# VISION-SJTU/USOT

Hardware: AMD Instinct MI355X
Metric: tracker FPS (255x255 search, ResNet-50) (higher is better)
Workload: dtype f32; 1 GPU; configs[1]: batch=1 ResNet-50(layer3)+neck, fused depthwise xcorr, cls/reg/memory heads (N_q=7), decode + PrRoIPool, fp32, 1 stream per GPU; search=255, template=127, streams=1, streams_per_gpu=1, weights=synthetic seed 0 (calibrated BN), no broadcast 0 B, hipgraph=True, devices_visible=1, sessions=1, hip_streams=1

## Files before the change

### usot_amd/csrc/smallm_f32.hip

```cpp
#include <hip/hip_runtime.h>
#include <stdint.h>
#include "usot_hip.h"
#include "common.h"

#ifndef USOT_RING
#define USOT_RING 8
#endif

namespace {

typedef float f32x4 __attribute__((ext_vector_type(4)));
typedef double f64x4 __attribute__((ext_vector_type(4)));
typedef unsigned int u32x4_t __attribute__((ext_vector_type(4)));
typedef unsigned int u32x2_t __attribute__((ext_vector_type(2)));
typedef _Float16 f16x8_t __attribute__((ext_vector_type(8)));

struct PwF {
    const float *t2, *w3p, *b3, *res, *w1p, *b1;
    float *y, *t, *ws;
    int M, act2;
    int parts = 0;
    const float *tbias = nullptr;
    int rparts = 0;
    const float *rbias = nullptr;
    int *ovf = nullptr;
};

template <int CBW, int RS, int RT, int PF, int BLO = 0>
struct GemmRing {
    static constexpr int N = CBW * RS;
    static_assert(BLO == 0 || (RS % 4 == 0 && PF % 2 == 0), "split-fp16: whole 64-k blocks, fragments in pairs");
    static_assert(PF <= N, "ring deeper than the work");
    f32x4 ring[PF];
    __device__ __forceinline__ f32x4 frag(const f32x4 *__restrict__ wf, int cb0, int r0, int n) const
    {
        return wf[((cb0 + n / RS) * RT + r0 + n % RS) * 64];
    }
    __device__ __forceinline__ void prefetch(const f32x4 *__restrict__ wf, int cb0, int r0)
    {
#pragma unroll
        for (int n = 0; n < PF; ++n) ring[n] = frag(wf, cb0, r0, n);
    }
    __device__ __forceinline__ void run(const f32x4 *__restrict__ wf, const float *bs, int cb0, int r0, f32x4 (&acc)[CBW])
    {
        constexpr int G = 4;
        const f32x4 zero = {0.f, 0.f, 0.f, 0.f};
        f32x4 part[CBW][2];
        BlockTotal tot[CBW];
#pragma unroll
        for (int u = 0; u < CBW; ++u) { part[u][0] = part[u][1] = zero; tot[u].clear(); }
        if constexpr (BLO > 0) {
            auto h = [](const f32x4 &v) { return __builtin_bit_cast(f16x8_t, v); };
#pragma unroll
            for (int n = 0; n < N; n += 2) {
                const int step = (r0 + n % RS) >> 1;
                const f32x4 bh = *(const f32x4 *)(bs + step * 16), bl = *(const f32x4 *)(bs + BLO + step * 16);
                const f32x4 ah = ring[n % PF], al = ring[(n + 1) % PF];
                if (n + PF < N) ring[n % PF] = frag(wf, cb0, r0, n + PF);
                if (n + 1 + PF < N) ring[(n + 1) % PF] = frag(wf, cb0, r0, n + 1 + PF);
                const int u = n / RS, rr = n % RS, g = rr / G, s = g & 1;
                const bool first = rr % G == 0;
                if (first && g >= 2) tot[u].add(part[u][s]);
                part[u][s] = __builtin_amdgcn_mfma_f32_16x16x32_f16(h(al), h(bh), first ? zero : part[u][s], 0, 0, 0);
                part[u][s] = __builtin_amdgcn_mfma_f32_16x16x32_f16(h(ah), h(bl), part[u][s], 0, 0, 0);
                part[u][s] = __builtin_amdgcn_mfma_f32_16x16x32_f16(h(ah), h(bh), part[u][s], 0, 0, 0);
            }
        } else {
#pragma unroll
        for (int n = 0; n < N; ++n) {
            const f32x4 b = *(const f32x4 *)(bs + (r0 + n % RS) * 16);
            const f32x4 a = ring[n % PF];
            if (n + PF < N) ring[n % PF] = frag(wf, cb0, r0, n + PF);
            const int u = n / RS, rr = n % RS, g = rr / G, s = g & 1;
            const bool first = rr % G == 0;
            if (first && g >= 2) tot[u].add(part[u][s]);
#pragma unroll
            for (int c = 0; c < 4; ++c)
                part[u][s] = __builtin_amdgcn_mfma_f32_16x16x4f32(a[c], b[c], (first && c == 0) ? zero : part[u][s], 0, 0, 0);
        }
        }
#pragma unroll
        for (int u = 0; u < CBW; ++u) {
            constexpr int GL = (RS - 1) / G;
            if (GL >= 1) tot[u].add(part[u][(GL & 1) ^ 1]);
            tot[u].add(part[u][GL & 1]);
            acc[u] = tot[u].get();
        }
    }
};

template <int CBW, int RS, int RT, int BLO = 0>
__device__ __forceinline__ void gemm_blocks(const f32x4 *__restrict__ wf, const float *bs, int cb0, int r0, f32x4 (&acc)[CBW])
{
    GemmRing<CBW, RS, RT, (CBW * RS < USOT_RING ? CBW * RS : USOT_RING), BLO> g;
    g.prefetch(wf, cb0, r0);
    g.run(wf, bs, cb0, r0, acc);
}

__device__ __forceinline__ void store_split4(char *row, int k, int plane, f32x4 v)
{
    v *= 8.0f;
    const uint32_t hi0 = usot_pack2_lp<true>(v[0], v[1]), hi1 = usot_pack2_lp<true>(v[2], v[3]);
    const usot_f16x2 h0 = __builtin_bit_cast(usot_f16x2, hi0), h1 = __builtin_bit_cast(usot_f16x2, hi1);
    const uint32_t lo0 = usot_pack2_lp<true>(v[0] - (float)h0[0], v[1] - (float)h0[1]);
    const uint32_t lo1 = usot_pack2_lp<true>(v[2] - (float)h1[0], v[3] - (float)h1[1]);
    *(u32x2_t *)(row + k * 2) = u32x2_t{hi0, hi1};
    *(u32x2_t *)(row + plane + k * 2) = u32x2_t{lo0, lo1};
}

__device__ __forceinline__ void note_not_finite(int *ovf, const f32x4 &a)
{
    if (!ovf) return;
    bool bad = false;
#pragma unroll
    for (int e = 0; e < 4; ++e) bad |= !(__builtin_fabsf(a[e]) <= 3.4028234664e38f);
    if (bad) __hip_atomic_store(ovf, 1, __ATOMIC_RELAXED, __HIP_MEMORY_SCOPE_AGENT);
}

template <int CM, int COT, int CN, int S, bool H16 = false>
__device__ __forceinline__ void pair_tail(const PwF &p, const float *Xs, float *Ys, float *Ps, int pt, int sl)
{
    constexpr int NW = 8, BM = 16;
    constexpr int CO = COT / S;
    constexpr int R1 = CM / 16, NB1 = CO / 16;
    constexpr int R2 = CO / 16, NB2 = CN / 16, R2T = COT / 16;
    constexpr int CBW1 = NB1 / NW;
    constexpr int KS = NB2 >= NW ? 1 : NW / NB2;
    constexpr int CBW2 = NB2 >= NW ? NB2 / NW : 1;
    constexpr int RS2 = R2 / KS;
    static_assert(NB1 % NW == 0 && (NB2 % NW == 0 || NW % NB2 == 0) && R2 % KS == 0, "shape");
    static_assert(S == 1 || KS == 1, "the sliced form keeps GEMM2's k range of a workgroup in one piece");
    constexpr int XP = CM + 4, YP = CO + 4, PP = CN + 4;
    const int tid = threadIdx.x, lane = tid & 63, wave = tid >> 6;
    const int l15 = lane & 15, quad = lane >> 4;
    const int m = pt * BM + l15;
    const bool mok = m < p.M;

    {
        f32x4 rr[CBW1], bb[CBW1], sc[H16 ? CBW1 : 1];
#pragma unroll
        for (int u = 0; u < CBW1; ++u) {
            const int cog = sl * CO + (wave * CBW1 + u) * 16 + quad * 4;
            if constexpr (H16) sc[u] = *(const f32x4 *)(p.w3p + (long)COT * CM + cog);
            rr[u] = mok ? *(const f32x4 *)(p.res + (long)m * COT + cog) : f32x4{0.f, 0.f, 0.f, 0.f};
            if (p.rparts > 1 && mok) {
                for (int q = 1; q < p.rparts; ++q) rr[u] += *(const f32x4 *)(p.res + ((long)q * p.M + m) * COT + cog);
                rr[u] += *(const f32x4 *)(p.rbias + cog);
            }
            bb[u] = *(const f32x4 *)(p.b3 + cog);
        }
        f32x4 acc[CBW1];
        gemm_blocks<CBW1, R1, R1, H16 ? CM / 2 : 0>((const f32x4 *)p.w3p + lane + (long)sl * NB1 * R1 * 64, Xs + l15 * XP + quad * 4, wave * CBW1, 0, acc);
#pragma unroll
        for (int u = 0; u < CBW1; ++u) {
            const int co = (wave * CBW1 + u) * 16 + quad * 4;
            if constexpr (H16) {
                acc[u] *= sc[u];
                note_not_finite(p.ovf, acc[u]);
            }
            f32x4 v = acc[u] + bb[u] + rr[u];
#pragma unroll
            for (int e = 0; e < 4; ++e) v[e] = fmaxf(v[e], 0.f);
            if (mok) *(f32x4 *)(p.y + (long)m * COT + sl * CO + co) = v;
            if constexpr (H16) store_split4((char *)(Ys + l15 * YP), co, CO * 2, v);
            else *(f32x4 *)(Ys + l15 * YP + co) = v;
        }
    }
    __syncthreads();

    const int ksl = KS > 1 ? wave / NB2 : 0;
    const int cb0 = KS > 1 ? wave % NB2 : wave * CBW2;
    f32x4 acc[CBW2];
    gemm_blocks<CBW2, RS2, R2T, H16 ? CO / 2 : 0>((const f32x4 *)p.w1p + lane + (long)sl * R2 * 64, Ys + l15 * YP + quad * 4, cb0, ksl * RS2, acc);
    if constexpr (H16) {
#pragma unroll
        for (int u = 0; u < CBW2; ++u) {
            acc[u] *= *(const f32x4 *)(p.w1p + (long)CN * COT + (cb0 + u) * 16 + quad * 4);
            note_not_finite(p.ovf, acc[u]);
        }
    }
    if constexpr (KS > 1) {
        const int cn = cb0 * 16 + quad * 4;
        if (ksl > 0) *(f32x4 *)(Ps + ((ksl - 1) * BM + l15) * PP + cn) = acc[0];
        __syncthreads();
        if (ksl > 0) return;
#pragma unroll
        for (int s = 1; s < KS; ++s) acc[0] += *(const f32x4 *)(Ps + ((s - 1) * BM + l15) * PP + cn);
    }
    if constexpr (S > 1) {
        const long bytes = (long)S * p.M * CN * 4;
        const __amdgpu_buffer_rsrc_t rs = __builtin_amdgcn_make_buffer_rsrc((void *)p.ws, 0, (int)(bytes > 0x7fffffffL ? 0x7fffffffL : bytes), 0x00020000);
#pragma unroll
        for (int u = 0; u < CBW2; ++u)
            if (mok) __builtin_amdgcn_raw_buffer_store_b128(__builtin_bit_cast(u32x4_t, acc[u]), rs,
                                                            (int)((((long)sl * p.M + m) * CN + (cb0 + u) * 16 + quad * 4) * 4), 0, 16);
        asm volatile("s_waitcnt vmcnt(0)" ::: "memory");
        __syncthreads();
        int *flag = (int *)Ps;
        if (tid == 0) {
            int *cnt = (int *)(p.ws + (long)S * p.M * CN) + pt;
            const int ticket = __hip_atomic_fetch_add(cnt, 1, __ATOMIC_RELAXED, __HIP_MEMORY_SCOPE_AGENT);
            const int last = ticket == S - 1;
            if (last) __hip_atomic_store(cnt, 0, __ATOMIC_RELAXED, __HIP_MEMORY_SCOPE_AGENT);
            *flag = last;
        }
        __syncthreads();
        if (!*flag || !mok) return;
#pragma unroll
        for (int u = 0; u < CBW2; ++u) {
            f32x4 sum = {0.f, 0.f, 0.f, 0.f};
#pragma unroll
            for (int q = 0; q < S; ++q)
                sum += __builtin_bit_cast(f32x4, __builtin_amdgcn_raw_buffer_load_b128(rs, (int)((((long)q * p.M + m) * CN + (cb0 + u) * 16 + quad * 4) * 4), 0, 16));
            acc[u] = sum;
        }
    }
#pragma unroll
    for (int u = 0; u < CBW2; ++u) {
        const int cn = (cb0 + u) * 16 + quad * 4;
        f32x4 v = acc[u] + *(const f32x4 *)(p.b1 + cn);
        if (p.act2 == USOT_ACT_RELU) {
#pragma unroll
            for (int e = 0; e < 4; ++e) v[e] = fmaxf(v[e], 0.f);
        }
        if (mok) *(f32x4 *)(p.t + (long)m * CN + cn) = v;
    }
}

template <int CN, int KSG> constexpr int ps_floats() { return KSG > 1 ? (KSG - 1) * 16 * (CN + 4) : 16; }

template <int CM, int COT, int CN, int S = 1, bool H16 = false>
__global__ __launch_bounds__(512) void pw_pair_f32_kernel(const PwF p)
{
    constexpr int NW = 8, BM = 16, XP = CM + 4, NB2 = CN / 16, KS = NB2 >= NW ? 1 : NW / NB2;
    __shared__ __attribute__((aligned(16))) float Xs[BM * XP];
    __shared__ __attribute__((aligned(16))) float Ys[BM * (COT / S + 4)];
    __shared__ __attribute__((aligned(16))) float Ps[ps_floats<CN, KS>()];
    const int tid = threadIdx.x;
    const int pt = S > 1 ? (int)blockIdx.x / S : (int)blockIdx.x, sl = S > 1 ? (int)blockIdx.x % S : 0;
    const int bm0 = pt * BM;
    if (p.parts > 1) {
        const long slab = (long)p.M * CM;
        for (int i = tid; i < BM * (CM / 4); i += NW * 64) {
            const int row = i / (CM / 4), c4 = i - row * (CM / 4);
            f32x4 v = {0.f, 0.f, 0.f, 0.f};
            if (bm0 + row < p.M) {
                const float *src = p.t2 + (long)(bm0 + row) * CM + c4 * 4;
                v = *(const f32x4 *)src;
                for (int q = 1; q < p.parts; ++q) v += *(const f32x4 *)(src + q * slab);
                v += *(const f32x4 *)(p.tbias + c4 * 4);
#pragma unroll
                for (int e = 0; e < 4; ++e) v[e] = fmaxf(v[e], 0.f);
            }
            if constexpr (H16) store_split4((char *)(Xs + row * XP), c4 * 4, CM * 2, v);
            else *(f32x4 *)(Xs + row * XP + c4 * 4) = v;
        }
    } else {
        for (int i = tid; i < BM * (CM / 4); i += NW * 64) {
            const int row = i / (CM / 4), c4 = i - row * (CM / 4);
            f32x4 v = {0.f, 0.f, 0.f, 0.f};
            if (bm0 + row < p.M) v = *(const f32x4 *)(p.t2 + (long)(bm0 + row) * CM + c4 * 4);
            if constexpr (H16) store_split4((char *)(Xs + row * XP), c4 * 4, CM * 2, v);
            else *(f32x4 *)(Xs + row * XP + c4 * 4) = v;
        }
    }
    __syncthreads();
    pair_tail<CM, COT, CN, S, H16>(p, Xs, Ys, Ps, pt, sl);
}

struct PwT {
    PwF pair;
    const float *x, *w2p, *b2;
    int H, W, OH, OW, pad_h, pad_w, dil_h, dil_w;
};

template <int CIN, int CM, int COT, int CN>
__global__ __launch_bounds__(512) void pw_triple_f32_kernel(const PwT q)
{
    constexpr int NW = 8, BM = 16, TAPS = 9, K0 = TAPS * CIN, RT0 = K0 / 16, NB0 = CM / 16;
    constexpr int KS0 = NW / NB0, RS0 = RT0 / KS0;
    static_assert(NB0 <= NW && NW % NB0 == 0 && RT0 % KS0 == 0, "conv2: one column block per wave group");
    constexpr int XP0 = K0 + 4, XP = CM + 4, NB2 = CN / 16, KS2 = NB2 >= NW ? 1 : NW / NB2;
    constexpr int PSF = ps_floats<CM, KS0>() > ps_floats<CN, KS2>() ? ps_floats<CM, KS0>() : ps_floats<CN, KS2>();
    extern __shared__ __attribute__((aligned(16))) float ldst[];
    float *X0 = ldst;
    float *Xs = X0 + BM * XP0;
    float *Ys = Xs + BM * XP;
    float *Ps = Ys + BM * (COT + 4);
    __shared__ int pix[BM][3];
    const PwF &p = q.pair;
    const int tid = threadIdx.x, lane = tid & 63, wave = tid >> 6;
    const int l15 = lane & 15, quad = lane >> 4;
    const int pt = blockIdx.x, bm0 = pt * BM;
    const int cb = wave % NB0, ksl = wave / NB0;
    const f32x4 *wf = (const f32x4 *)q.w2p + lane;
    GemmRing<1, RS0, RT0, (RS0 < USOT_RING ? RS0 : USOT_RING)> g;
    g.prefetch(wf, cb, ksl * RS0);
    if (tid < BM) {
        const int mm = bm0 + tid;
        if (mm < p.M) {
            const int P = q.OH * q.OW, n = mm / P, r = mm - n * P, oh = r / q.OW;
            pix[tid][0] = n * q.H;
            pix[tid][1] = oh - q.pad_h;
            pix[tid][2] = (r - oh * q.OW) - q.pad_w;
        } else {
            pix[tid][0] = -1;
        }
    }
    __syncthreads();
    for (int i = tid; i < BM * TAPS * (CIN / 4); i += NW * 64) {
        const int c4 = i % (CIN / 4), t = (i / (CIN / 4)) % TAPS, row = i / (TAPS * (CIN / 4));
        f32x4 v = {0.f, 0.f, 0.f, 0.f};
        if (pix[row][0] >= 0) {
            const int ih = pix[row][1] + (t / 3) * q.dil_h, iw = pix[row][2] + (t % 3) * q.dil_w;
            if ((unsigned)ih < (unsigned)q.H && (unsigned)iw < (unsigned)q.W)
                v = *(const f32x4 *)(q.x + ((long)(pix[row][0] + ih) * q.W + iw) * CIN + c4 * 4);
        }
        *(f32x4 *)(X0 + row * XP0 + t * CIN + c4 * 4) = v;
    }
    const f32x4 b2 = *(const f32x4 *)(q.b2 + cb * 16 + quad * 4);
    __syncthreads();
    f32x4 acc[1];
    g.run(wf, X0 + l15 * XP0 + quad * 4, cb, ksl * RS0, acc);
    if constexpr (KS0 > 1) {
        if (ksl > 0) *(f32x4 *)(Ps + ((ksl - 1) * BM + l15) * (CM + 4) + cb * 16 + quad * 4) = acc[0];
        __syncthreads();
        if (ksl == 0) {
#pragma unroll
            for (int s2 = 1; s2 < KS0; ++s2) acc[0] += *(const f32x4 *)(Ps + ((s2 - 1) * BM + l15) * (CM + 4) + cb * 16 + quad * 4);
        }
    }
    if (ksl == 0) {
        f32x4 v = acc[0] + b2;
#pragma unroll
        for (int e = 0; e < 4; ++e) v[e] = fmaxf(v[e], 0.f);
        *(f32x4 *)(Xs + l15 * XP + cb * 16 + quad * 4) = v;
    }
    __syncthreads();
    pair_tail<CM, COT, CN, 1>(p, Xs, Ys, Ps, pt, 0);
}

template <int CM, int CO, int CN, int S = 1, bool H16 = false> int launch(hipStream_t s, const PwF &p)
{
    hipLaunchKernelGGL((pw_pair_f32_kernel<CM, CO, CN, S, H16>), dim3(((p.M + 15) / 16) * S), dim3(512), 0, s, p);
    return hipGetLastError() == hipSuccess ? USOT_OK : USOT_ELAUNCH;
}

template <int CIN, int CM, int CO, int CN> int launch_triple(hipStream_t s, const PwT &q)
{
    const int usot_dv = usot_device_slot();
    if (usot_dv < 0) return USOT_ESTATE;
    constexpr int NB2 = CN / 16, KS2 = NB2 >= 8 ? 1 : 8 / NB2, KS0 = 8 / (CM / 16);
    constexpr int PSF = ps_floats<CM, KS0>() > ps_floats<CN, KS2>() ? ps_floats<CM, KS0>() : ps_floats<CN, KS2>();
    const size_t lds = (size_t)(16 * (9 * CIN + 4) + 16 * (CM + 4) + 16 * (CO + 4) + PSF) * sizeof(float);
    static bool raised_d[USOT_MAX_DEV] = {};
    bool &raised = raised_d[usot_dv];
    if (lds > 64 * 1024 && !raised) {
        if (hipFuncSetAttribute((const void *)pw_triple_f32_kernel<CIN, CM, CO, CN>, hipFuncAttributeMaxDynamicSharedMemorySize, (int)lds) != hipSuccess)
            return USOT_ELAUNCH;
        raised = true;
    }
    hipLaunchKernelGGL((pw_triple_f32_kernel<CIN, CM, CO, CN>), dim3((q.pair.M + 15) / 16), dim3(512), lds, s, q);
    return hipGetLastError() == hipSuccess ? USOT_OK : USOT_ELAUNCH;
}

int slices(int M, int CM, int CN)
{
    if (CM == 128 && CN == 128 && M <= 2 * 961) return 4;
    if (CM == 256 && CN == 256 && M <= 1200) return 4;
    return 1;
}

struct Pw1 {
    const float *x, *wp, *b, *res;
    float *y;
    int M, act;
};

template <int K, int N, int S, int PFD = USOT_RING>
__global__ __launch_bounds__(512) void pw_single_f32_kernel(const Pw1 p)
{
    constexpr int NW = 8, BM = 16;
    constexpr int RT = K / 16, NB = N / 16 / S;
    constexpr int KS = NB >= NW ? 1 : NW / NB, CBW = NB >= NW ? NB / NW : 1, RS = RT / KS;
    static_assert((NB % NW == 0 || NW % NB == 0) && RT % KS == 0, "shape");
    constexpr int XP = K + 4, PP = NB * 16 + 4;
    extern __shared__ __attribute__((aligned(16))) float lds1[];
    float *Xs = lds1;
    float *Ps = lds1 + BM * XP;

    const int tid = threadIdx.x, lane = tid & 63, wave = tid >> 6;
    const int l15 = lane & 15, quad = lane >> 4;
    const int pt = (int)blockIdx.x / S, sl = (int)blockIdx.x % S;
    const int bm0 = pt * BM, m = bm0 + l15;
    const bool mok = m < p.M;
    const int ksl = KS > 1 ? wave / NB : 0;
    const int cb0 = KS > 1 ? wave % NB : wave * CBW;
    const f32x4 *wf = (const f32x4 *)p.wp + lane + (long)sl * NB * RT * 64;
    GemmRing<CBW, RS, RT, (CBW * RS < PFD ? CBW * RS : PFD)> g;
    g.prefetch(wf, cb0, ksl * RS);
    for (int i = tid; i < BM * (K / 4); i += NW * 64) {
        const int row = i / (K / 4), c4 = i - row * (K / 4);
        f32x4 v = {0.f, 0.f, 0.f, 0.f};
        if (bm0 + row < p.M) v = *(const f32x4 *)(p.x + (long)(bm0 + row) * K + c4 * 4);
        *(f32x4 *)(Xs + row * XP + c4 * 4) = v;
    }
    f32x4 rr[CBW], bb[CBW];
#pragma unroll
    for (int u = 0; u < CBW; ++u) {
        const int n = (sl * NB + cb0 + u) * 16 + quad * 4;
        rr[u] = (mok && p.res && ksl == 0) ? *(const f32x4 *)(p.res + (long)m * N + n) : f32x4{0.f, 0.f, 0.f, 0.f};
        bb[u] = *(const f32x4 *)(p.b + n);
    }
    __syncthreads();
    f32x4 acc[CBW];
    g.run(wf, Xs + l15 * XP + quad * 4, cb0, ksl * RS, acc);
    if constexpr (KS > 1) {
        if (ksl > 0) *(f32x4 *)(Ps + ((ksl - 1) * BM + l15) * PP + cb0 * 16 + quad * 4) = acc[0];
        __syncthreads();
        if (ksl > 0) return;
#pragma unroll
        for (int s2 = 1; s2 < KS; ++s2) acc[0] += *(const f32x4 *)(Ps + ((s2 - 1) * BM + l15) * PP + cb0 * 16 + quad * 4);
    }
#pragma unroll
    for (int u = 0; u < CBW; ++u) {
        f32x4 v = acc[u] + bb[u] + rr[u];
        if (p.act == USOT_ACT_RELU) {
#pragma unroll
            for (int e = 0; e < 4; ++e) v[e] = fmaxf(v[e], 0.f);
        }
        if (mok) *(f32x4 *)(p.y + (long)m * N + (sl * NB + cb0 + u) * 16 + quad * 4) = v;
    }
}

template <int K, int N, int S> int launch1(hipStream_t s, const Pw1 &p)
{
    const int usot_dv = usot_device_slot();
    if (usot_dv < 0) return USOT_ESTATE;
    constexpr int NB = N / 16 / S, KS = NB >= 8 ? 1 : 8 / NB;
    const size_t lds = (size_t)(16 * (K + 4) + (KS > 1 ? (KS - 1) * 16 * (NB * 16 + 4) : 0)) * sizeof(float);
    if (lds > 64 * 1024) {
        static bool raised_d[USOT_MAX_DEV] = {};
    bool &raised = raised_d[usot_dv];
        if (!raised) {
            if (hipFuncSetAttribute((const void *)pw_single_f32_kernel<K, N, S>, hipFuncAttributeMaxDynamicSharedMemorySize, (int)lds) != hipSuccess)
                return USOT_ELAUNCH;
            raised = true;
        }
    }
    hipLaunchKernelGGL((pw_single_f32_kernel<K, N, S>), dim3(((p.M + 15) / 16) * S), dim3(512), lds, s, p);
    return hipGetLastError() == hipSuccess ? USOT_OK : USOT_ELAUNCH;
}

struct PwC {
    const float *x, *wp, *b, *res;
    float *y;
    int M, H, W, OH, OW, pad_h, pad_w, dil_h, dil_w, act;
};

template <int CIN, int N, int S>
__global__ __launch_bounds__(512) void stream_conv3x3_f32_kernel(const PwC p)
{
    constexpr int NW = 8, BM = 16, TAPS = 9, K = TAPS * CIN;
    constexpr int RT = K / 16, NB = N / 16 / S;
    constexpr int KS = NB >= NW ? 1 : NW / NB, CBW = NB >= NW ? NB / NW : 1, RS = RT / KS;
    static_assert((NB % NW == 0 || NW % NB == 0) && RT % KS == 0, "shape");
    constexpr int XP = K + 4, PP = NB * 16 + 4;
    extern __shared__ __attribute__((aligned(16))) float ldsc[];
    float *Xs = ldsc;
    float *Ps = ldsc + BM * XP;
    __shared__ int pix[BM][3];

    const int tid = threadIdx.x, lane = tid & 63, wave = tid >> 6;
    const int l15 = lane & 15, quad = lane >> 4;
    const int pt = (int)blockIdx.x / S, sl = (int)blockIdx.x % S;
    const int bm0 = pt * BM, m = bm0 + l15;
    const bool mok = m < p.M;
    const int ksl = KS > 1 ? wave / NB : 0;
    const int cb0 = KS > 1 ? wave % NB : wave * CBW;
    const f32x4 *wf = (const f32x4 *)p.wp + lane + (long)sl * NB * RT * 64;
    GemmRing<CBW, RS, RT, (CBW * RS < USOT_RING ? CBW * RS : USOT_RING)> g;
    g.prefetch(wf, cb0, ksl * RS);
    if (tid < BM) {
        const int mm = bm0 + tid;
        if (mm < p.M) {
            const int P = p.OH * p.OW, n = mm / P, r = mm - n * P, oh = r / p.OW;
            pix[tid][0] = n * p.H;
            pix[tid][1] = oh - p.pad_h;
            pix[tid][2] = (r - oh * p.OW) - p.pad_w;
        } else {
            pix[tid][0] = -1;
        }
    }
    __syncthreads();
    for (int i = tid; i < BM * TAPS * (CIN / 4); i += NW * 64) {
        const int c4 = i % (CIN / 4), t = (i / (CIN / 4)) % TAPS, row = i / (TAPS * (CIN / 4));
        f32x4 v = {0.f, 0.f, 0.f, 0.f};
        if (pix[row][0] >= 0) {
            const int ih = pix[row][1] + (t / 3) * p.dil_h, iw = pix[row][2] + (t % 3) * p.dil_w;
            if ((unsigned)ih < (unsigned)p.H && (unsigned)iw < (unsigned)p.W)
                v = *(const f32x4 *)(p.x + ((long)(pix[row][0] + ih) * p.W + iw) * CIN + c4 * 4);
        }
        *(f32x4 *)(Xs + row * XP + t * CIN + c4 * 4) = v;
    }
    f32x4 rr[CBW], bb[CBW];
#pragma unroll
    for (int u = 0; u < CBW; ++u) {
        const int n = (sl * NB + cb0 + u) * 16 + quad * 4;
        rr[u] = (mok && p.res && ksl == 0) ? *(const f32x4 *)(p.res + (long)m * N + n) : f32x4{0.f, 0.f, 0.f, 0.f};
        bb[u] = *(const f32x4 *)(p.b + n);
    }
    __syncthreads();
    f32x4 acc[CBW];
    g.run(wf, Xs + l15 * XP + quad * 4, cb0, ksl * RS, acc);
    if constexpr (KS > 1) {
        if (ksl > 0) *(f32x4 *)(Ps + ((ksl - 1) * BM + l15) * PP + cb0 * 16 + quad * 4) = acc[0];
        __syncthreads();
        if (ksl > 0) return;
#pragma unroll
        for (int s2 = 1; s2 < KS; ++s2) acc[0] += *(const f32x4 *)(Ps + ((s2 - 1) * BM + l15) * PP + cb0 * 16 + quad * 4);
    }
#pragma unroll
    for (int u = 0; u < CBW; ++u) {
        f32x4 v = acc[u] + bb[u] + rr[u];
        if (p.act == USOT_ACT_RELU) {
#pragma unroll
            for (int e = 0; e < 4; ++e) v[e] = fmaxf(v[e], 0.f);
        }
        if (mok) *(f32x4 *)(p.y + (long)m * N + (sl * NB + cb0 + u) * 16 + quad * 4) = v;
    }
}

template <int CIN, int N, int S> int launch3(hipStream_t s, const PwC &p)
{
    const int usot_dv = usot_device_slot();
    if (usot_dv < 0) return USOT_ESTATE;
    constexpr int K = 9 * CIN, NB = N / 16 / S, KS = NB >= 8 ? 1 : 8 / NB;
    const size_t lds = (size_t)(16 * (K + 4) + (KS > 1 ? (KS - 1) * 16 * (NB * 16 + 4) : 0)) * sizeof(float);
    static bool raised_d[USOT_MAX_DEV] = {};
    bool &raised = raised_d[usot_dv];
    if (lds > 64 * 1024 && !raised) {
        if (hipFuncSetAttribute((const void *)stream_conv3x3_f32_kernel<CIN, N, S>, hipFuncAttributeMaxDynamicSharedMemorySize, (int)lds) != hipSuccess)
            return USOT_ELAUNCH;
        raised = true;
    }
    hipLaunchKernelGGL((stream_conv3x3_f32_kernel<CIN, N, S>), dim3(((p.M + 15) / 16) * S), dim3(512), lds, s, p);
    return hipGetLastError() == hipSuccess ? USOT_OK : USOT_ELAUNCH;
}

}

extern "C" int usot_pw_pair_f32_supported(int CM, int CO, int CN)
{
    return (CM == 64 && CO == 256 && (CN == 64 || CN == 128)) || (CM == 128 && CO == 512 && (CN == 128 || CN == 256)) ||
           (CM == 256 && CO == 1024 && CN == 256);
}

extern "C" int64_t usot_pw_pair_f32_ws_floats(int M, int CM, int CO, int CN)
{
    (void)CO;
    const int S = slices(M, CM, CN);
    return S > 1 ? (int64_t)S * M * CN + (M + 15) / 16 : 0;
}

static int pw_pair_f32_launch(void *stream, const usot_pw_pair_desc *d, bool split16);

extern "C" int usot_pw_pair_f32(void *stream, const usot_pw_pair_desc *d) { return pw_pair_f32_launch(stream, d, false); }

extern "C" int usot_pw_pair_f32s(void *stream, const usot_pw_pair_desc *d) { return pw_pair_f32_launch(stream, d, true); }

extern "C" int usot_pw_pair_f32s_supported(int CM, int CO, int CN) { return CM == 256 && CO == 1024 && CN == 256; }

static int pw_pair_f32_launch(void *stream, const usot_pw_pair_desc *d, bool split16)
{
    if (!d || !d->t2 || !d->w3p || !d->b3 || !d->res || !d->w1 || !d->b1 || !d->y || !d->t || d->M <= 0) return USOT_EINVAL;
    if (d->act2 != USOT_ACT_NONE && d->act2 != USOT_ACT_RELU) return USOT_EINVAL;
    const uintptr_t al = (uintptr_t)d->t2 | (uintptr_t)d->w3p | (uintptr_t)d->b3 | (uintptr_t)d->res | (uintptr_t)d->w1 |
                         (uintptr_t)d->b1 | (uintptr_t)d->y | (uintptr_t)d->t | (uintptr_t)d->ws;
    if (al & 15) return USOT_EINVAL;
    if (d->t2_parts > 1 && (!d->t2_bias || ((uintptr_t)d->t2_bias & 15) || d->t2_parts > 16)) return USOT_EINVAL;
    PwF p{(const float *)d->t2, (const float *)d->w3p, d->b3, (const float *)d->res, (const float *)d->w1, d->b1,
          (float *)d->y, (float *)d->t, (float *)d->ws, d->M, d->act2};
    p.parts = d->t2_parts > 1 ? d->t2_parts : 0;
    p.tbias = d->t2_bias;
    if (d->res_parts > 1 && (!d->res_bias || ((uintptr_t)d->res_bias & 15) || d->res_parts > 16)) return USOT_EINVAL;
    p.rparts = d->res_parts > 1 ? d->res_parts : 0;
    p.rbias = d->res_bias;
    if ((uintptr_t)d->ovf & 3) return USOT_EINVAL;
    p.ovf = split16 ? d->ovf : nullptr;
    hipStream_t s = (hipStream_t)stream;
    const bool sliced = slices(d->M, d->CM, d->CN) > 1 && d->ws;
    if (split16) {
        if (d->CM == 256 && d->CO == 1024 && d->CN == 256 && sliced) return launch<256, 1024, 256, 4, true>(s, p);
        return USOT_EINVAL;
    }
    if (d->CM == 64 && d->CO == 256 && d->CN == 64) return launch<64, 256, 64>(s, p);
    if (d->CM == 64 && d->CO == 256 && d->CN == 128) return launch<64, 256, 128>(s, p);
    if (d->CM == 128 && d->CO == 512 && d->CN == 128) return sliced ? launch<128, 512, 128, 4>(s, p) : launch<128, 512, 128>(s, p);
    if (d->CM == 128 && d->CO == 512 && d->CN == 256) return launch<128, 512, 256>(s, p);
    if (d->CM == 256 && d->CO == 1024 && d->CN == 256 && sliced) return launch<256, 1024, 256, 4>(s, p);
    return USOT_EINVAL;
}

extern "C" int usot_pw_single_f32_supported(int K, int N)
{
    return (K == 1024 && N == 256) || (K == 256 && N == 1024) || (K == 512 && N == 128) || (K == 128 && N == 512);
}

extern "C" int usot_pw_single_f32(void *stream, const float *x, const float *wp, const float *b, const float *res, float *y,
                                  int M, int K, int N, int act)
{
    if (!x || !wp || !b || !y || M <= 0 || (act != USOT_ACT_NONE && act != USOT_ACT_RELU)) return USOT_EINVAL;
    if (((uintptr_t)x | (uintptr_t)wp | (uintptr_t)b | (uintptr_t)res | (uintptr_t)y) & 15) return USOT_EINVAL;
    const Pw1 p{x, wp, b, res, y, M, act};
    hipStream_t s = (hipStream_t)stream;
    if (K == 1024 && N == 256) return launch1<1024, 256, 4>(s, p);
    if (K == 256 && N == 1024) return launch1<256, 1024, 8>(s, p);
    if (K == 512 && N == 128) return launch1<512, 128, 2>(s, p);
    if (K == 128 && N == 512) return launch1<128, 512, 4>(s, p);
    return USOT_EINVAL;
}

extern "C" int usot_stream_conv3x3_f32_supported(int Cin, int N) { return (Cin == 256 && N == 256) || (Cin == 128 && N == 128); }

extern "C" int usot_stream_conv3x3_f32(void *stream, const float *x, const float *wp, const float *b, const float *res, float *y,
                                       int Nb, int H, int W, int Cin, int OH, int OW, int N, int pad_h, int pad_w, int dil_h, int dil_w,
                                       int act)
{
    if (!x || !wp || !b || !y || Nb <= 0 || (act != USOT_ACT_NONE && act != USOT_ACT_RELU)) return USOT_EINVAL;
    if (((uintptr_t)x | (uintptr_t)wp | (uintptr_t)b | (uintptr_t)res | (uintptr_t)y) & 15) return USOT_EINVAL;
    if (OH != H + 2 * pad_h - 2 * dil_h || OW != W + 2 * pad_w - 2 * dil_w || OH <= 0 || OW <= 0) return USOT_EINVAL;
    const PwC p{x, wp, b, res, y, Nb * OH * OW, H, W, OH, OW, pad_h, pad_w, dil_h, dil_w, act};
    hipStream_t s = (hipStream_t)stream;
    if (Cin == 256 && N == 256) return launch3<256, 256, 4>(s, p);
    if (Cin == 128 && N == 128) return launch3<128, 128, 4>(s, p);
    return USOT_EINVAL;
}

extern "C" int usot_pw_triple_f32_supported(int Cin, int CM, int CO, int CN)
{
    return (Cin == 64 && CM == 64 && CO == 256 && (CN == 64 || CN == 128)) || (Cin == 128 && CM == 128 && CO == 512 && CN == 128);
}

extern "C" int usot_pw_triple_f32(void *stream, const float *x, const float *w2p, const float *b2, const usot_pw_pair_desc *d,
                                  int Nb, int H, int W, int Cin, int OH, int OW, int pad_h, int pad_w, int dil_h, int dil_w)
{
    if (!x || !w2p || !b2 || !d || !d->w3p || !d->b3 || !d->res || !d->w1 || !d->b1 || !d->y || !d->t) return USOT_EINVAL;
    if (!usot_pw_triple_f32_supported(Cin, d->CM, d->CO, d->CN) || d->M != Nb * OH * OW || d->M <= 0) return USOT_EINVAL;
    if (OH != H + 2 * pad_h - 2 * dil_h || OW != W + 2 * pad_w - 2 * dil_w) return USOT_EINVAL;
    if (d->act2 != USOT_ACT_NONE && d->act2 != USOT_ACT_RELU) return USOT_EINVAL;
    const uintptr_t al = (uintptr_t)x | (uintptr_t)w2p | (uintptr_t)b2 | (uintptr_t)d->w3p | (uintptr_t)d->b3 | (uintptr_t)d->res |
                         (uintptr_t)d->w1 | (uintptr_t)d->b1 | (uintptr_t)d->y | (uintptr_t)d->t;
    if (al & 15) return USOT_EINVAL;
    PwT q;
    q.pair = PwF{nullptr, (const float *)d->w3p, d->b3, (const float *)d->res, (const float *)d->w1, d->b1, (float *)d->y,
                 (float *)d->t, nullptr, d->M, d->act2};
    q.x = x; q.w2p = w2p; q.b2 = b2;
    q.H = H; q.W = W; q.OH = OH; q.OW = OW; q.pad_h = pad_h; q.pad_w = pad_w; q.dil_h = dil_h; q.dil_w = dil_w;
    hipStream_t s = (hipStream_t)stream;
    if (Cin == 128) return launch_triple<128, 128, 512, 128>(s, q);
    if (d->CN == 64) return launch_triple<64, 64, 256, 64>(s, q);
    return launch_triple<64, 64, 256, 128>(s, q);
}
```

Before: 1198 frames/s.

## Pin weight-ring prefetch with sched barriers and hoist pair-GEMM head loads

Adds sched_barrier pins around the weight-fragment ring loads so the compiler cannot sink or reorder the prefetches. The LDS B-fragments are now software-pipelined one step ahead. In the fused pointwise pair kernels, the first GEMM's weight ring, residual, bias and scale loads move before the input staging and barrier. The second GEMM's ring is prefetched right after the first GEMM runs. The aim is to hide global weight-load latency behind LDS staging and MFMA work, at the cost of more live registers and a higher risk of spills or lower occupancy.

```diff
diff --git a/usot_amd/csrc/smallm_f32.hip b/usot_amd/csrc/smallm_f32.hip
--- a/usot_amd/csrc/smallm_f32.hip
+++ b/usot_amd/csrc/smallm_f32.hip
@@ -5,6 +5,13 @@
 
 #ifndef USOT_RING
 #define USOT_RING 8
+#endif
+#ifdef USOT_RING_UNPINNED
+#define USOT_RING_PIN() ((void)0)
+static constexpr bool kPinned = false;
+#else
+#define USOT_RING_PIN() __builtin_amdgcn_sched_barrier(0)
+static constexpr bool kPinned = true;
 #endif
 
 namespace {
@@ -40,6 +47,7 @@
     {
 #pragma unroll
         for (int n = 0; n < PF; ++n) ring[n] = frag(wf, cb0, r0, n);
+        USOT_RING_PIN();
     }
     __device__ __forceinline__ void run(const f32x4 *__restrict__ wf, const float *bs, int cb0, int r0, f32x4 (&acc)[CBW])
     {
@@ -51,13 +59,18 @@
         for (int u = 0; u < CBW; ++u) { part[u][0] = part[u][1] = zero; tot[u].clear(); }
         if constexpr (BLO > 0) {
             auto h = [](const f32x4 &v) { return __builtin_bit_cast(f16x8_t, v); };
+            auto bfrag = [&](int n, int lo) { return *(const f32x4 *)(bs + lo + ((r0 + n % RS) >> 1) * 16); };
+            f32x4 bhn, bln;
+            if (kPinned) { bhn = bfrag(0, 0); bln = bfrag(0, BLO); }
 #pragma unroll
             for (int n = 0; n < N; n += 2) {
-                const int step = (r0 + n % RS) >> 1;
-                const f32x4 bh = *(const f32x4 *)(bs + step * 16), bl = *(const f32x4 *)(bs + BLO + step * 16);
+                const f32x4 bh = kPinned ? bhn : bfrag(n, 0), bl = kPinned ? bln : bfrag(n, BLO);
+                if (kPinned && n + 2 < N) { bhn = bfrag(n + 2, 0); bln = bfrag(n + 2, BLO); }
                 const f32x4 ah = ring[n % PF], al = ring[(n + 1) % PF];
+                USOT_RING_PIN();
                 if (n + PF < N) ring[n % PF] = frag(wf, cb0, r0, n + PF);
                 if (n + 1 + PF < N) ring[(n + 1) % PF] = frag(wf, cb0, r0, n + 1 + PF);
+                USOT_RING_PIN();
                 const int u = n / RS, rr = n % RS, g = rr / G, s = g & 1;
                 const bool first = rr % G == 0;
                 if (first && g >= 2) tot[u].add(part[u][s]);
@@ -66,11 +79,17 @@
                 part[u][s] = __builtin_amdgcn_mfma_f32_16x16x32_f16(h(ah), h(bh), part[u][s], 0, 0, 0);
             }
         } else {
+        auto bfrag = [&](int n) { return *(const f32x4 *)(bs + (r0 + n % RS) * 16); };
+        f32x4 bn;
+        if (kPinned) bn = bfrag(0);
 #pragma unroll
         for (int n = 0; n < N; ++n) {
-            const f32x4 b = *(const f32x4 *)(bs + (r0 + n % RS) * 16);
+            const f32x4 b = kPinned ? bn : bfrag(n);
+            if (kPinned && n + 1 < N) bn = bfrag(n + 1);
             const f32x4 a = ring[n % PF];
+            USOT_RING_PIN();
             if (n + PF < N) ring[n % PF] = frag(wf, cb0, r0, n + PF);
+            USOT_RING_PIN();
             const int u = n / RS, rr = n % RS, g = rr / G, s = g & 1;
             const bool first = rr % G == 0;
             if (first && g >= 2) tot[u].add(part[u][s]);
@@ -89,10 +108,13 @@
     }
 };
 
+template <int CBW, int RS, int RT, int BLO = 0, int PFD = USOT_RING>
+using RingOf = GemmRing<CBW, RS, RT, (CBW * RS < PFD ? CBW * RS : PFD), BLO>;
+
 template <int CBW, int RS, int RT, int BLO = 0>
 __device__ __forceinline__ void gemm_blocks(const f32x4 *__restrict__ wf, const float *bs, int cb0, int r0, f32x4 (&acc)[CBW])
 {
-    GemmRing<CBW, RS, RT, (CBW * RS < USOT_RING ? CBW * RS : USOT_RING), BLO> g;
+    RingOf<CBW, RS, RT, BLO> g;
     g.prefetch(wf, cb0, r0);
     g.run(wf, bs, cb0, r0, acc);
 }
@@ -117,8 +139,38 @@
     if (bad) __hip_atomic_store(ovf, 1, __ATOMIC_RELAXED, __HIP_MEMORY_SCOPE_AGENT);
 }
 
+template <int CM, int COT, int S, bool H16>
+struct PairHead {
+    static constexpr int NW = 8, BM = 16, CO = COT / S, R1 = CM / 16, NB1 = CO / 16, CBW1 = NB1 / NW;
+    RingOf<CBW1, R1, R1, H16 ? CM / 2 : 0> g;
+    f32x4 rr[CBW1], bb[CBW1], sc[H16 ? CBW1 : 1];
+    __device__ __forceinline__ const f32x4 *wf(const PwF &p, int sl) const
+    {
+        return (const f32x4 *)p.w3p + (threadIdx.x & 63) + (long)sl * NB1 * R1 * 64;
+    }
+    __device__ __forceinline__ void issue(const PwF &p, int pt, int sl)
+    {
+        const int lane = threadIdx.x & 63, wave = threadIdx.x >> 6, quad = lane >> 4;
+        const int m = pt * BM + (lane & 15);
+        const bool mok = m < p.M;
+        g.prefetch(wf(p, sl), wave * CBW1, 0);
+#pragma unroll
+        for (int u = 0; u < CBW1; ++u) {
+            const int cog = sl * CO + (wave * CBW1 + u) * 16 + quad * 4;
+            if constexpr (H16) sc[u] = *(const f32x4 *)(p.w3p + (long)COT * CM + cog);
+            rr[u] = mok ? *(const f32x4 *)(p.res + (long)m * COT + cog) : f32x4{0.f, 0.f, 0.f, 0.f};
+            if (p.rparts > 1 && mok) {
+                for (int q = 1; q < p.rparts; ++q) rr[u] += *(const f32x4 *)(p.res + ((long)q * p.M + m) * COT + cog);
+                rr[u] += *(const f32x4 *)(p.rbias + cog);
+            }
+            bb[u] = *(const f32x4 *)(p.b3 + cog);
+        }
+        USOT_RING_PIN();
+    }
+};
+
 template <int CM, int COT, int CN, int S, bool H16 = false>
-__device__ __forceinline__ void pair_tail(const PwF &p, const float *Xs, float *Ys, float *Ps, int pt, int sl)
+__device__ __forceinline__ void pair_tail(const PwF &p, PairHead<CM, COT, S, H16> &hd, const float *Xs, float *Ys, float *Ps, int pt, int sl)
 {
     constexpr int NW = 8, BM = 16;
     constexpr int CO = COT / S;
@@ -136,7 +188,15 @@
     const int m = pt * BM + l15;
     const bool mok = m < p.M;
 
+#ifndef USOT_RING_UNPINNED
+    const int ksl = KS > 1 ? wave / NB2 : 0;
+    const int cb0 = KS > 1 ? wave % NB2 : wave * CBW2;
+    const f32x4 *wf2 = (const f32x4 *)p.w1p + lane + (long)sl * R2 * 64;
+    RingOf<CBW2, RS2, R2T, H16 ? CO / 2 : 0> g2;
+#endif
+
     {
+#ifdef USOT_RING_UNPINNED
         f32x4 rr[CBW1], bb[CBW1], sc[H16 ? CBW1 : 1];
 #pragma unroll
         for (int u = 0; u < CBW1; ++u) {
@@ -151,6 +211,14 @@
         }
         f32x4 acc[CBW1];
         gemm_blocks<CBW1, R1, R1, H16 ? CM / 2 : 0>((const f32x4 *)p.w3p + lane + (long)sl * NB1 * R1 * 64, Xs + l15 * XP + quad * 4, wave * CBW1, 0, acc);
+#else
+        const auto &rr = hd.rr;
+        const auto &bb = hd.bb;
+        const auto &sc = hd.sc;
+        f32x4 acc[CBW1];
+        hd.g.run(hd.wf(p, sl), Xs + l15 * XP + quad * 4, wave * CBW1, 0, acc);
+        g2.prefetch(wf2, cb0, ksl * RS2);
+#endif
 #pragma unroll
         for (int u = 0; u < CBW1; ++u) {
             const int co = (wave * CBW1 + u) * 16 + quad * 4;
@@ -168,10 +236,14 @@
     }
     __syncthreads();
 
+    f32x4 acc[CBW2];
+#ifdef USOT_RING_UNPINNED
     const int ksl = KS > 1 ? wave / NB2 : 0;
     const int cb0 = KS > 1 ? wave % NB2 : wave * CBW2;
-    f32x4 acc[CBW2];
     gemm_blocks<CBW2, RS2, R2T, H16 ? CO / 2 : 0>((const f32x4 *)p.w1p + lane + (long)sl * R2 * 64, Ys + l15 * YP + quad * 4, cb0, ksl * RS2, acc);
+#else
+    g2.run(wf2, Ys + l15 * YP + quad * 4, cb0, ksl * RS2, acc);
+#endif
     if constexpr (H16) {
 #pragma unroll
         for (int u = 0; u < CBW2; ++u) {
@@ -239,6 +311,8 @@
     const int tid = threadIdx.x;
     const int pt = S > 1 ? (int)blockIdx.x / S : (int)blockIdx.x, sl = S > 1 ? (int)blockIdx.x % S : 0;
     const int bm0 = pt * BM;
+    PairHead<CM, COT, S, H16> hd;
+    if (kPinned) hd.issue(p, pt, sl);
     if (p.parts > 1) {
         const long slab = (long)p.M * CM;
         for (int i = tid; i < BM * (CM / 4); i += NW * 64) {
@@ -265,7 +339,7 @@
         }
     }
     __syncthreads();
-    pair_tail<CM, COT, CN, S, H16>(p, Xs, Ys, Ps, pt, sl);
+    pair_tail<CM, COT, CN, S, H16>(p, hd, Xs, Ys, Ps, pt, sl);
 }
 
 struct PwT {
@@ -294,7 +368,7 @@
     const int pt = blockIdx.x, bm0 = pt * BM;
     const int cb = wave % NB0, ksl = wave / NB0;
     const f32x4 *wf = (const f32x4 *)q.w2p + lane;
-    GemmRing<1, RS0, RT0, (RS0 < USOT_RING ? RS0 : USOT_RING)> g;
+    RingOf<1, RS0, RT0> g;
     g.prefetch(wf, cb, ksl * RS0);
     if (tid < BM) {
         const int mm = bm0 + tid;
@@ -322,6 +396,8 @@
     __syncthreads();
     f32x4 acc[1];
     g.run(wf, X0 + l15 * XP0 + quad * 4, cb, ksl * RS0, acc);
+    PairHead<CM, COT, 1, false> hd;
+    if (kPinned) hd.issue(p, pt, 0);
     if constexpr (KS0 > 1) {
         if (ksl > 0) *(f32x4 *)(Ps + ((ksl - 1) * BM + l15) * (CM + 4) + cb * 16 + quad * 4) = acc[0];
         __syncthreads();
@@ -337,7 +413,7 @@
         *(f32x4 *)(Xs + l15 * XP + cb * 16 + quad * 4) = v;
     }
     __syncthreads();
-    pair_tail<CM, COT, CN, 1>(p, Xs, Ys, Ps, pt, 0);
+    pair_tail<CM, COT, CN, 1>(p, hd, Xs, Ys, Ps, pt, 0);
 }
 
 template <int CM, int CO, int CN, int S = 1, bool H16 = false> int launch(hipStream_t s, const PwF &p)
@@ -397,7 +473,7 @@
     const int ksl = KS > 1 ? wave / NB : 0;
     const int cb0 = KS > 1 ? wave % NB : wave * CBW;
     const f32x4 *wf = (const f32x4 *)p.wp + lane + (long)sl * NB * RT * 64;
-    GemmRing<CBW, RS, RT, (CBW * RS < PFD ? CBW * RS : PFD)> g;
+    RingOf<CBW, RS, RT, 0, PFD> g;
     g.prefetch(wf, cb0, ksl * RS);
     for (int i = tid; i < BM * (K / 4); i += NW * 64) {
         const int row = i / (K / 4), c4 = i - row * (K / 4);
@@ -479,7 +555,7 @@
     const int ksl = KS > 1 ? wave / NB : 0;
     const int cb0 = KS > 1 ? wave % NB : wave * CBW;
     const f32x4 *wf = (const f32x4 *)p.wp + lane + (long)sl * NB * RT * 64;
-    GemmRing<CBW, RS, RT, (CBW * RS < USOT_RING ? CBW * RS : USOT_RING)> g;
+    RingOf<CBW, RS, RT> g;
     g.prefetch(wf, cb0, ksl * RS);
     if (tid < BM) {
         const int mm = bm0 + tid;
```

After: 1256 frames/s (median of 6 runs). 1.05x the previous value.
